# conceptofmind/vit-flax

Measured on NVIDIA B200. Metric: images/sec ViT-B/16 224 bf16 fwd at 1/2/4/8 B200; % tensor-pipe peak, higher is better.
Workload: dtype bf16

## Files before the change

vit_flax_b200/csrc/api.cu:

```cuda
#include <algorithm>
#include <cmath>
#include <cstdlib>
#include <map>
#include <memory>
#include <string>
#include <vector>

#include <cuda_fp16.h>

#include "common.h"

namespace vb {
namespace {

constexpr int DIM_HEAD = 64;

struct Leaf {
  std::string path;
  std::vector<int64_t> shape;
  float* dev = nullptr;
  bool set = false;
  int64_t numel() const {
    int64_t n = 1;
    for (auto s : shape) n *= s;
// ... 430 lines not shown
                    const AttnRecord* rec = nullptr) {
  const auto& c = m->cfg;
  const int D = c.dim, I = m->inner, T = m->T;
  const int R = batch * T;
  const ActMaps* am;
  int rc;
  if ((rc = get_act_maps(m, batch, &am))) return rc;
  const int cg_qkv = gemm_tc_tile_mode(R, 3 * I), cg_d = gemm_tc_tile_mode(R, D), cg_ff1 = gemm_tc_tile_mode(R, c.mlp_dim);
  LnFold out_a, out_b, in_a, in_b;
  out_a.x16 = out_b.x16 = m->xn_h.p;
  out_a.stats = in_a.stats = reinterpret_cast<float2*>(m->stats_a.p);
  out_b.stats = in_b.stats = reinterpret_cast<float2*>(m->stats_b.p);
  out_a.slots = out_b.slots = in_a.slots = in_b.slots = 2 * ceil_div(D, cg_d == 64 ? 64 : GEMM_BN);
  in_a.eps = in_b.eps = m->eps;
  if (m->im2col && out_a.slots % (2 * ceil_div(D, GEMM_BN)) == 0 && (reinterpret_cast<uintptr_t>(images) & 15) == 0) {
    mark(m, st, VITB200_CAT_GEMM_PATCH);
    if ((rc = patch_embed_im2col(m, st, images, batch, &out_a))) return rc;
  } else {
    mark(m, st, VITB200_CAT_PATCHIFY);
    if ((rc = launch_patchify(st, images, m->patches_h.p, batch, c.image_h, c.image_w, c.channels,
                              c.patch_h, c.patch_w, m->K0pad, m->dt, m->nchw, m->cls_off))) return rc;
    mark(m, st, VITB200_CAT_GEMM_PATCH);
    if ((rc = launch_gemm_tc(st, am->patches, m->patch.map(cg_d), &am->c_x, leaf_ptr(m, m->patch.leaf_bias), m->x.p,
                             R, D, m->K0pad, VITB200_EPI_TOKENS_LN, leaf_ptr(m, m->leaf_pos), T, m->dt, cg_d,
                             Dropout(), m->cls_off, leaf_ptr(m, m->leaf_cls), out_a))) return rc;
  }
  const bool tail = cls_tail(m, rec);
  for (int l = 0; l < c.depth; ++l) {
    Layer& L = m->layers[l];
    const bool cls_rows = tail && l + 1 == c.depth;
    const int M = cls_rows ? batch : R;
    const CUtensorMap& a_o = cls_rows ? am->o_cls : am->o;
    const CUtensorMap& c_x = cls_rows ? am->c_x_cls : am->c_x;
    mark(m, st, VITB200_CAT_GEMM_QKV);
    in_a.c = L.qkv.ln_c;
    if ((rc = launch_gemm_tc(st, am->xn, L.qkv.map_ln(cg_qkv), &am->c_qkv, L.qkv.ln_d, m->qkv_h.p, R, 3 * I, D,
                             VITB200_EPI_LN_STORE_16, nullptr, 0, m->dt, cg_qkv, Dropout(), m->cls_off, nullptr, in_a))) return rc;
    mark(m, st, VITB200_CAT_ATTENTION);
    if ((rc = attention_layer(m, st, batch, l, rec, cls_rows ? 1 : 0))) return rc;
    mark(m, st, VITB200_CAT_GEMM_OUT);
    if ((rc = launch_gemm_tc(st, a_o, L.out.map(cg_d), &c_x, leaf_ptr(m, L.out.leaf_bias), m->x.p, M, D, I,
                             VITB200_EPI_RESID_LN, nullptr, 0, m->dt, cg_d, Dropout(), m->cls_off, nullptr, out_b))) return rc;
    mark(m, st, VITB200_CAT_GEMM_FF1);
    in_b.c = L.ff1.ln_c;
    if ((rc = launch_gemm_tc(st, am->xn, L.ff1.map_ln(cg_ff1), &am->c_hid, L.ff1.ln_d, m->hid_h.p, M, c.mlp_dim, D,
                             VITB200_EPI_LN_GELU_16, nullptr, 0, m->dt, cg_ff1, Dropout(), m->cls_off, nullptr, in_b))) return rc;
    mark(m, st, VITB200_CAT_GEMM_FF2);
    if (l + 1 < c.depth) {
      if ((rc = launch_gemm_tc(st, am->h, L.ff2.map(cg_d), &am->c_x, leaf_ptr(m, L.ff2.leaf_bias), m->x.p, R, D, c.mlp_dim,
                               VITB200_EPI_RESID_LN, nullptr, 0, m->dt, cg_d, Dropout(), m->cls_off, nullptr, out_a))) return rc;
    } else {
      if ((rc = launch_gemm_tc(st, am->h, L.ff2.map(cg_d), &c_x, leaf_ptr(m, L.ff2.leaf_bias), m->x.p, M, D, c.mlp_dim,
                               VITB200_EPI_BIAS_RESID_F32, nullptr, 0, m->dt, cg_d))) return rc;
    }
  }
  return forward_head(m, st, am, batch, logits);
}

int forward_tc(vitb200_model* m, cudaStream_t st, const float* images, int batch, float* logits,
               const AttnRecord* rec = nullptr) {
  if (m->fold) return forward_tc_fold(m, st, images, batch, logits, rec);
  const auto& c = m->cfg;
  const int D = c.dim, I = m->inner, T = m->T;
  const int R = batch * T;
  const ActMaps* am;
  int rc;
  if ((rc = get_act_maps(m, batch, &am))) return rc;
  const int cgp = gemm_tc_tile_mode(R, D);
  const int cg_qkv = gemm_tc_tile_mode(R, 3 * I), cg_d = gemm_tc_tile_mode(R, D), cg_ff1 = gemm_tc_tile_mode(R, c.mlp_dim);
  const int ln_dt = m->fp8 ? VITB200_DT_E4M3 : m->dt;
  if (m->im2col && (reinterpret_cast<uintptr_t>(images) & 15) == 0) {
    mark(m, st, VITB200_CAT_GEMM_PATCH);
    if ((rc = patch_embed_im2col(m, st, images, batch, nullptr))) return rc;
  } else {
    mark(m, st, VITB200_CAT_PATCHIFY);
// ... 1232 lines not shown
```

vit_flax_b200/csrc/gemm_tc.cu:

```cuda
#include <cstdlib>

#include "common.h"
#include "ptx.cuh"

namespace vb {

namespace {

constexpr int BM = GEMM_BM, BN = GEMM_BN, BK = GEMM_BK;
constexpr int UMMA_K = 16;
constexpr int A_BYTES = BM * BK * 2;
template <int kCG> struct Cfg {
  static constexpr int CL = kCG == 64 ? 1 : kCG;
  static constexpr int BN_ = kCG == 64 ? 64 : BN;
  static constexpr int MMA_CG = CL == 1 ? 1 : 2;
  static constexpr int STAGES = kCG == 64 ? 6 : (CL == 1 ? 3 : 5);
  static constexpr int B_ROWS = BN_ / MMA_CG;
  static constexpr int B_LOAD_ROWS = BN_ / CL;
  static constexpr int B_BYTES = B_ROWS * BK * 2;
  static constexpr int STAGE_BYTES = A_BYTES + B_BYTES;
  static constexpr int TILE_M = BM * MMA_CG;
  static constexpr int PAIRS = kCG == 4 ? 2 : 1;
  static constexpr int TMEM_COLS = BN_ == 64 ? 128 : 512;
};
constexpr int NUM_EPI_WARPS = 8;
constexpr int NUM_THREADS = 128 + NUM_EPI_WARPS * 32;
constexpr int SLAB_BYTES = BM * 128;
template <int kEpi> __host__ __device__ constexpr int slabs_per_group() { return kEpi == VITB200_EPI_RESID_LN ? 3 : 2; }
template <int kCG, int kEpi> __host__ __device__ constexpr int num_stages() {
  return Cfg<kCG>::STAGES - (kEpi == VITB200_EPI_RESID_LN ? 1 : 0);
}
template <int kCG, int kEpi = VITB200_EPI_STORE_16> constexpr int smem_bytes() {
  return num_stages<kCG, kEpi>() * Cfg<kCG>::STAGE_BYTES + 2 * slabs_per_group<kEpi>() * SLAB_BYTES + 1024  +
         256 ;
}

__device__ __forceinline__ float gelu_tanh_fast(float x) {
  const float k0 = 0.7978845608028654f, k1 = 0.044715f;
  float u = k0 * x * fmaf(k1 * x, x, 1.0f);
  return 0.5f * x * (1.0f + tanh_approx(u));
}

__device__ __forceinline__ unsigned long long gelu_tanh_fast2(unsigned long long x2) {
  const unsigned long long kA = pack_f32x2(0.7978845608028654f * 0.044715f, 0.7978845608028654f * 0.044715f);
  const unsigned long long kB = pack_f32x2(0.7978845608028654f, 0.7978845608028654f);
  const unsigned long long half2 = pack_f32x2(0.5f, 0.5f);
  const unsigned long long t2 = mul_f32x2(x2, x2);
  const unsigned long long u2 = mul_f32x2(fma_f32x2(t2, kA, kB), x2);
  float u0, u1;
  unpack_f32x2(u2, u0, u1);
  const unsigned long long th2 = pack_f32x2(tanh_approx(u0), tanh_approx(u1));
  const unsigned long long hx2 = mul_f32x2(x2, half2);
  return fma_f32x2(th2, hx2, hx2);
}

template <int kEpi, int kDT, int kCG, bool kDrop, bool kMN = false>
__global__ void __launch_bounds__(NUM_THREADS, 1)
gemm_tc_kernel(const __grid_constant__ CUtensorMap tmA,
               const __grid_constant__ CUtensorMap tmB,
               const __grid_constant__ CUtensorMap tmC,
               const float* __restrict__ bias, void* __restrict__ Cout,
               int M, int N, int K, const float* __restrict__ aux, int tpi, int dbg, Dropout drop, int cls_off,
               const float* __restrict__ cls, LnFold ln, const float* __restrict__ wscale) {
  constexpr bool kF8 = (kDT == DT_E4M3);
  constexpr int kODT = kF8 ? DT_F16 : kDT;
  constexpr int KB = kF8 ? 128 : BK;
  static_assert(!kF8 || (!kMN && !kDrop), "E4M3 operands: K-major, no dropout");
  constexpr bool kOut8 = (kEpi == VITB200_EPI_BIAS_GELU_E4M3);
  constexpr bool kOut16 = (kEpi == VITB200_EPI_STORE_16 || kEpi == VITB200_EPI_BIAS_GELU_16 || kEpi == VITB200_EPI_BIAS_16 ||
                           kEpi == VITB200_EPI_BIAS_PRE_GELU_16 || kEpi == VITB200_EPI_LN_STORE_16 ||
                           kEpi == VITB200_EPI_LN_GELU_16);
  constexpr bool kLnIn = (kEpi == VITB200_EPI_LN_STORE_16 || kEpi == VITB200_EPI_LN_GELU_16);
  constexpr bool kLnOut = (kEpi == VITB200_EPI_RESID_LN || kEpi == VITB200_EPI_TOKENS_LN);
  constexpr bool kLoadX = (kEpi == VITB200_EPI_RESID_LN);
  constexpr bool kTokens = (kEpi == VITB200_EPI_TOKENS_F32 || kEpi == VITB200_EPI_TOKENS_LN);
  constexpr int SPG = slabs_per_group<kEpi>();
  constexpr bool kDual = (kEpi == VITB200_EPI_BIAS_PRE_GELU_16);
  constexpr bool kDirect = (kEpi == VITB200_EPI_PATCH_F32);
  constexpr int SLAB_COLS = (kOut16 || kOut8) ? 64 : 32;
  constexpr int SLABS_PER_TILE = Cfg<kCG>::BN_ / SLAB_COLS;
  constexpr int STAGES = num_stages<kCG, kEpi>(), B_BYTES = Cfg<kCG>::B_BYTES;
  constexpr int STAGE_BYTES = Cfg<kCG>::STAGE_BYTES, TILE_M = Cfg<kCG>::TILE_M;
  constexpr int MMA_CG = Cfg<kCG>::MMA_CG, PAIRS = Cfg<kCG>::PAIRS, CL = Cfg<kCG>::CL;
  constexpr int BN = Cfg<kCG>::BN_, TMEM_COLS = Cfg<kCG>::TMEM_COLS;
  const uint32_t crank = CL == 1 ? 0u : cluster_ctarank();
  const uint32_t rank = crank & 1u, pair = crank >> 1;
  const uint32_t lead = crank & ~1u;
  const int tile0 = int(blockIdx.x) / CL;
  const int tile_step = int(gridDim.x) / CL;

  extern __shared__ uint8_t smem_raw[];
  const uint32_t smem_base = (smem_u32(smem_raw) + 1023u) & ~1023u;
  const uint32_t sA = smem_base;
  const uint32_t sB = smem_base + STAGES * A_BYTES;
  const uint32_t sSlab = smem_base + STAGES * STAGE_BYTES;
  const uint32_t bars = sSlab + 2 * SPG * SLAB_BYTES;
  auto full_bar = [&](int s) { return bars + 8u * s; };
  auto empty_bar = [&](int s) { return bars + 8u * (STAGES + s); };
  auto tfull_bar = [&](int s) { return bars + 8u * (2 * STAGES + s); };
  auto tempty_bar = [&](int s) { return bars + 8u * (2 * STAGES + 2 + s); };
  const uint32_t tmem_slot = bars + 8u * (2 * STAGES + 4);
  auto xfull_bar = [&](int g, int b) { return bars + 8u * (2 * STAGES + 5 + g * 3 + b); };
  uint32_t* tmem_slot_ptr =
      reinterpret_cast<uint32_t*>(smem_raw + (tmem_slot - smem_u32(smem_raw)));

  const int warp = threadIdx.x >> 5;
  const int lane = threadIdx.x & 31;
  const int m_tiles = ((M + TILE_M - 1) / TILE_M + PAIRS - 1) / PAIRS;
  const int n_tiles = (N + BN - 1) / BN;
  const int num_kb = (K + KB - 1) / KB;
  const int splits = (kEpi == VITB200_EPI_BIAS_RESID_F32 && tpi > 1) ? tpi : 1;
  const int kb_per = (num_kb + splits - 1) / splits;
  const int mn_tiles = m_tiles * n_tiles;
  const int num_tiles = mn_tiles * splits;

  if (warp == 0 && lane == 0) {
    prefetch_tmap(&tmA);
    prefetch_tmap(&tmB);
    if constexpr (!kDirect) prefetch_tmap(&tmC);
  }
  if (warp == 1 && lane == 0) {
    for (int s = 0; s < STAGES; ++s) {
      mbar_init(full_bar(s), 1);
      mbar_init(empty_bar(s), PAIRS);
    }
    for (int s = 0; s < 2; ++s) {
      mbar_init(tfull_bar(s), 1);
      mbar_init(tempty_bar(s), NUM_EPI_WARPS * MMA_CG);
    }
    if constexpr (kLoadX)
      for (int i = 0; i < 6; ++i) mbar_init(xfull_bar(i / 3, i % 3), 1);
    fence_barrier_init();
  }
  if (warp == 2) tmem_alloc<MMA_CG>(tmem_slot, TMEM_COLS);
  tc_fence_before();
  if constexpr (CL != 1) cluster_sync_all(); else __syncthreads();
  tc_fence_after();
  const uint32_t tmem_base = *tmem_slot_ptr;
  pdl_launch_dependents();
  pdl_wait();

  if (warp == 0) {
    if (elect_one()) {
      int stage = 0;
      uint32_t phase = 0;
      for (int tile = tile0; tile < num_tiles; tile += tile_step) {
        const int sp = tile / mn_tiles, t2 = tile - sp * mn_tiles;
        const int m_blk = t2 / n_tiles, n_blk = t2 % n_tiles;
        const int kb0 = sp * kb_per, kb1 = min(num_kb, kb0 + kb_per);
        const int a_row = (m_blk * PAIRS + int(pair)) * TILE_M + int(rank) * BM;
        const int b_row = n_blk * BN + int(rank) * Cfg<kCG>::B_ROWS + int(pair) * Cfg<kCG>::B_LOAD_ROWS;
        for (int kb = kb0; kb < kb1; ++kb) {
          mbar_wait(empty_bar(stage), phase ^ 1u);
          if (dbg & 1) {
            if (rank == 0) mbar_arrive(full_bar(stage));
          } else if constexpr (CL == 1) {
            mbar_arrive_expect_tx(full_bar(stage), STAGE_BYTES);
            if constexpr (kMN) {
#pragma unroll
              for (int j = 0; j < BM / 64; ++j)
                tma_load_2d(sA + stage * A_BYTES + j * 8192, &tmA, full_bar(stage), a_row + j * 64, kb * BK);
#pragma unroll
              for (int j = 0; j < Cfg<kCG>::B_ROWS / 64; ++j)
// ... 52 lines not shown
          for (int k = 0; k < BK / UMMA_K; ++k) {
            if constexpr (kF8)
              umma_f8_ss<MMA_CG>(d_tmem, umma_desc_k_sw128(a0 + k * UMMA_K * 2), umma_desc_k_sw128(b0 + k * UMMA_K * 2),
                                 idesc, (kb != kb0 || k != 0) ? 1u : 0u);
            else if constexpr (kMN)
              umma_bf16_ss<MMA_CG>(d_tmem, umma_desc_mn_sw128_wide(a0 + k * UMMA_K * 128, 8192),
                                   umma_desc_mn_sw128_wide(b0 + k * UMMA_K * 128, 8192), idesc,
                                   (kb != kb0 || k != 0) ? 1u : 0u);
            else
            umma_bf16_ss<MMA_CG>(d_tmem, umma_desc_k_sw128(a0 + k * UMMA_K * 2),
                              umma_desc_k_sw128(b0 + k * UMMA_K * 2), idesc,
                              (kb != kb0 || k != 0) ? 1u : 0u);
          }
          if constexpr (CL != 1) umma_commit_cg2_mc(empty_bar(stage), all_mask);
          else umma_commit(empty_bar(stage));
          if (++stage == STAGES) { stage = 0; phase ^= 1u; }
        }
        if constexpr (CL != 1) umma_commit_cg2_mc(tfull_bar(acc), pair_mask);
        else umma_commit(tfull_bar(acc));
        acc ^= 1;
        if (acc == 0) acc_phase ^= 1u;
      }
    }
    __syncwarp();
  } else if (warp >= 4) {
    const int ew = warp - 4;
    const int q = ew & 3;
    const int grp = ew >> 2;
    const bool leader = (q == 0 && lane == 0);
    const int lrow = q * 32 + lane;
    int acc = 0;
    uint32_t acc_phase = 0;
    int buf = 0;
    int ld_tile = tile0, ld_s = grp, ld_issued = 0, x_used = 0;
    auto issue_x_load = [&]() {
      while (ld_tile < num_tiles) {
        if (ld_s < SLABS_PER_TILE && (ld_tile % n_tiles) * BN + ld_s * SLAB_COLS < N) break;
        ld_tile += tile_step;
        ld_s = grp;
      }
      if (ld_tile >= num_tiles) return;
      const int lm = ld_tile / n_tiles, lnb = ld_tile % n_tiles;
      const int b = ld_issued % 3;
      mbar_arrive_expect_tx(xfull_bar(grp, b), SLAB_BYTES);
      tma_load_2d(sSlab + uint32_t(grp * SPG + b) * SLAB_BYTES, &tmC, xfull_bar(grp, b), lnb * BN + ld_s * SLAB_COLS,
                  (lm * PAIRS + int(pair)) * TILE_M + int(rank) * BM);
      ++ld_issued;
      ld_s += 2;
    };
    if constexpr (kLoadX) {
      if (leader) { issue_x_load(); issue_x_load(); }
    }
    for (int tile = tile0; tile < num_tiles; tile += tile_step) {
      const int sp = tile / mn_tiles, t2 = tile - sp * mn_tiles;
      const int m_blk = t2 / n_tiles, n_blk = t2 % n_tiles;
      const int m_row0 = (m_blk * PAIRS + int(pair)) * TILE_M + int(rank) * BM;
      float ln_rstd = 0.f, ln_rm = 0.f;
      if constexpr (kLnIn) {
        if (m_row0 + lrow < M) {
          const float2* sp2 = ln.stats + int64_t(m_row0 + lrow) * ln.slots;
          float s1 = 0.f, s2 = 0.f;
          const float4* sp4 = reinterpret_cast<const float4*>(sp2);
          const int npair = (ln.slots & 1) ? 0 : ln.slots >> 1;
          if (ln.slots & 1) {
            for (int i = 0; i < ln.slots; ++i) { const float2 v = __ldg(sp2 + i); s1 += v.x; s2 += v.y; }
          }
          for (int i = 0; i < npair; i += 4) {
            float4 a[4];
#pragma unroll
            for (int u = 0; u < 4; ++u) a[u] = i + u < npair ? __ldg(sp4 + i + u) : make_float4(0.f, 0.f, 0.f, 0.f);
#pragma unroll
            for (int u = 0; u < 4; ++u)
              if (i + u < npair) { s1 += a[u].x; s2 += a[u].y; s1 += a[u].z; s2 += a[u].w; }
          }
          const float inv_d = 1.0f / float(K);
          const float mean = s1 * inv_d;
          ln_rstd = rsqrtf(fmaxf(s2 * inv_d - mean * mean, 0.f) + ln.eps);
          ln_rm = ln_rstd * mean;
        }
      }
      float st1 = 0.f, st2 = 0.f;
      mbar_wait(tfull_bar(acc), acc_phase);
      tc_fence_after();
      const uint32_t t_row = tmem_base + (uint32_t(q * 32) << 16) + uint32_t(acc * BN);

      if constexpr (kDirect) {
        const int row = m_row0 + lrow;
        const bool row_ok = row < M;
        const int b = row / tpi, t = row - b * tpi;
        float* crow_base = reinterpret_cast<float*>(Cout) + (int64_t(b) * (tpi + cls_off) + cls_off + t) * N;
        const float* pos_row = aux + int64_t(cls_off + t) * N;
#pragma unroll 1
        for (int chunk = 0; chunk < BN / 64; ++chunk) {
          const int n0 = n_blk * BN + grp * (BN / 2) + chunk * 32;
          if (n0 >= N) break;
          uint32_t r[32];
          tmem_ld_32x32b_x32(t_row + uint32_t(grp * (BN / 2) + chunk * 32), r);
          tmem_ld_wait();
          if (row_ok) {
#pragma unroll
            for (int j = 0; j < 8; ++j) {
              if (n0 + j * 4 < N) {
                const float4 b4 = __ldg(reinterpret_cast<const float4*>(bias + n0 + j * 4));
                const float4 p4 = __ldg(reinterpret_cast<const float4*>(pos_row + n0 + j * 4));
                float4 o;
                o.x = __uint_as_float(r[j * 4 + 0]) + b4.x + p4.x;
                o.y = __uint_as_float(r[j * 4 + 1]) + b4.y + p4.y;
                o.z = __uint_as_float(r[j * 4 + 2]) + b4.z + p4.z;
                o.w = __uint_as_float(r[j * 4 + 3]) + b4.w + p4.w;
                if constexpr (kDrop)
                  dropout4(drop, (int64_t(b) * (tpi + cls_off) + cls_off + t) * N + n0 + j * 4, o.x, o.y, o.z, o.w);
                *reinterpret_cast<float4*>(crow_base + n0 + j * 4) = o;
                if (cls != nullptr && t == 0) {
                  const float4 c4 = __ldg(reinterpret_cast<const float4*>(cls + n0 + j * 4));
                  const float4 q4 = __ldg(reinterpret_cast<const float4*>(aux + n0 + j * 4));
                  float4 z = make_float4(c4.x + q4.x, c4.y + q4.y, c4.z + q4.z, c4.w + q4.w);
                  const int64_t e0 = int64_t(b) * (tpi + 1) * N + n0 + j * 4;
                  if constexpr (kDrop) dropout4(drop, e0, z.x, z.y, z.z, z.w);
                  *reinterpret_cast<float4*>(reinterpret_cast<float*>(Cout) + e0) = z;
                }
              }
            }
          }
        }
      } else {
#pragma unroll 1
        for (int s = grp; s < SLABS_PER_TILE; s += 2) {
          const int n0 = n_blk * BN + s * SLAB_COLS;
          if (n0 >= N || (dbg & 4)) break;
          const uint32_t slab = sSlab + uint32_t(grp * SPG + (kLoadX ? x_used % 3 : buf)) * SLAB_BYTES;
          if constexpr (kLoadX) {
            mbar_wait(xfull_bar(grp, x_used % 3), uint32_t(x_used / 3) & 1u);
          } else {
            if (leader) { if constexpr (kDual) tma_store_wait_read<0>(); else tma_store_wait_read<1>(); }
            named_bar_sync(1 + grp, 128);
          }
          const uint32_t srow = slab + uint32_t(lrow) * 128u;
          const int sw = lrow & 7;
          const uint32_t srow2 = sSlab + uint32_t(grp * 2 + (buf ^ 1)) * SLAB_BYTES + uint32_t(lrow) * 128u;
          if constexpr (kOut16) {
#pragma unroll
            for (int half = 0; half < 2; ++half) {
              uint32_t r[32];
              tmem_ld_32x32b_x32(t_row + uint32_t(s * SLAB_COLS + half * 32), r);
              tmem_ld_wait();
#pragma unroll
              for (int j = 0; j < 4; ++j) {
                float v[8];
#pragma unroll
                for (int e = 0; e < 8; ++e) v[e] = __uint_as_float(r[j * 8 + e]);
                if constexpr (kF8) {
                  const int nb = n0 + half * 32 + j * 8;
                  if (nb < N) {
                    const float4 w0 = __ldg(reinterpret_cast<const float4*>(wscale + nb));
                    const float4 w1 = __ldg(reinterpret_cast<const float4*>(wscale + nb + 4));
                    v[0] *= w0.x; v[1] *= w0.y; v[2] *= w0.z; v[3] *= w0.w;
                    v[4] *= w1.x; v[5] *= w1.y; v[6] *= w1.z; v[7] *= w1.w;
                  }
                }
                if constexpr (kEpi == VITB200_EPI_BIAS_16 || kDual) {
                  const int nb = n0 + half * 32 + j * 8;
                  if (nb < N) {
                    const float4 b0 = __ldg(reinterpret_cast<const float4*>(bias + nb));
                    const float4 b1 = __ldg(reinterpret_cast<const float4*>(bias + nb + 4));
// ... 69 lines not shown
              tmem_ld_32x32b_x32(t_row + uint32_t(s * SLAB_COLS + half * 32), r);
              tmem_ld_wait();
#pragma unroll
              for (int j = 0; j < 2; ++j) {
                uint32_t q[4];
#pragma unroll
                for (int h = 0; h < 2; ++h) {
                  const int nb = n0 + half * 32 + j * 16 + h * 8;
                  float4 w0 = make_float4(0.f, 0.f, 0.f, 0.f), w1 = w0, b0 = w0, b1 = w0;
                  if (nb < N) {
                    w0 = __ldg(reinterpret_cast<const float4*>(wscale + nb));
                    w1 = __ldg(reinterpret_cast<const float4*>(wscale + nb + 4));
                    b0 = __ldg(reinterpret_cast<const float4*>(bias + nb));
                    b1 = __ldg(reinterpret_cast<const float4*>(bias + nb + 4));
                  }
                  const float ws[8] = {w0.x, w0.y, w0.z, w0.w, w1.x, w1.y, w1.z, w1.w};
                  const float bb[8] = {b0.x, b0.y, b0.z, b0.w, b1.x, b1.y, b1.z, b1.w};
                  float v[8];
#pragma unroll
                  for (int e = 0; e < 8; e += 2) {
                    const int c = j * 16 + h * 8 + e;
                    const unsigned long long y2 = fma_f32x2(pack_f32x2(__uint_as_float(r[c]), __uint_as_float(r[c + 1])),
                                                            pack_f32x2(ws[e], ws[e + 1]), pack_f32x2(bb[e], bb[e + 1]));
                    unpack_f32x2(gelu_tanh_fast2(y2), v[e], v[e + 1]);
                  }
                  q[h * 2] = pack4_e4m3(v[0], v[1], v[2], v[3]);
                  q[h * 2 + 1] = pack4_e4m3(v[4], v[5], v[6], v[7]);
                }
                const uint32_t lin = uint32_t(lrow) * 64u + uint32_t(half * 2 + j) * 16u;
                st_shared_v4(slab + (lin ^ (((lin >> 7) & 3u) << 4)), q[0], q[1], q[2], q[3]);
              }
            }
          } else {
            uint32_t r[32];
            tmem_ld_32x32b_x32(t_row + uint32_t(s * SLAB_COLS), r);
            const int tok = kTokens ? (m_row0 + lrow) % tpi : 0;
            const bool cls_row = kTokens && cls != nullptr && tok == 0;
            const float* pos_row = aux + int64_t(tok) * N;
            uint16_t* x16_row = kLnOut ? static_cast<uint16_t*>(ln.x16) + int64_t(m_row0 + lrow) * N : nullptr;
            const bool row_ok = m_row0 + lrow < M;
            uint32_t hx[8];
            tmem_ld_wait();
#pragma unroll
            for (int j = 0; j < 8; ++j) {
              const int nb = n0 + j * 4;
              float4 b4 = make_float4(0.f, 0.f, 0.f, 0.f);
              if (nb < N && sp == 0 && bias != nullptr) b4 = __ldg(reinterpret_cast<const float4*>((cls_row ? cls : bias) + nb));
              float o0 = __uint_as_float(r[j * 4 + 0]), o1 = __uint_as_float(r[j * 4 + 1]);
              float o2 = __uint_as_float(r[j * 4 + 2]), o3 = __uint_as_float(r[j * 4 + 3]);
              if constexpr (kF8) {
                if (nb < N) {
                  const float4 w4 = __ldg(reinterpret_cast<const float4*>(wscale + nb));
                  o0 *= w4.x; o1 *= w4.y; o2 *= w4.z; o3 *= w4.w;
                }
              }
              if constexpr (kTokens) {
                if (cls_row) o0 = o1 = o2 = o3 = 0.f;
                if (nb < N) {
                  const float4 p4 = __ldg(reinterpret_cast<const float4*>(pos_row + nb));
                  b4.x += p4.x; b4.y += p4.y; b4.z += p4.z; b4.w += p4.w;
                }
              }
              o0 += b4.x; o1 += b4.y; o2 += b4.z; o3 += b4.w;
              if constexpr (kDrop && kTokens)
                dropout4(drop, int64_t(m_row0 + lrow) * N + nb, o0, o1, o2, o3);
              if constexpr (kDrop && kEpi == VITB200_EPI_BIAS_RESID_F32)
                dropout4(drop, int64_t(m_row0 + lrow) * N + nb, o0, o1, o2, o3);
              if constexpr (kLoadX) {
                const float4 xo = ld_shared_v4f(srow + (uint32_t(j ^ sw) << 4));
                o0 += xo.x; o1 += xo.y; o2 += xo.z; o3 += xo.w;
              }
              st_shared_v4(srow + (uint32_t(j ^ sw) << 4), __float_as_uint(o0), __float_as_uint(o1),
                           __float_as_uint(o2), __float_as_uint(o3));
              if constexpr (kLnOut) {
                st1 += (o0 + o1) + (o2 + o3);
                st2 = fmaf(o0, o0, fmaf(o1, o1, fmaf(o2, o2, fmaf(o3, o3, st2))));
                hx[(j & 3) * 2] = pack2<kDT>(o0, o1);
                hx[(j & 3) * 2 + 1] = pack2<kDT>(o2, o3);
                if ((j & 3) == 3 && row_ok) {
                  if (nb + 4 <= N && (N & 15) == 0)
                    asm volatile("st.global.v8.b32 [%0], {%1, %2, %3, %4, %5, %6, %7, %8};" ::"l"(x16_row + nb - 12), "r"(hx[0]), "r"(hx[1]),
                                 "r"(hx[2]), "r"(hx[3]), "r"(hx[4]), "r"(hx[5]), "r"(hx[6]), "r"(hx[7]) : "memory");
                  else {
                    if (nb - 4 <= N) *reinterpret_cast<uint4*>(x16_row + nb - 12) = make_uint4(hx[0], hx[1], hx[2], hx[3]);
                    if (nb + 4 <= N) *reinterpret_cast<uint4*>(x16_row + nb - 4) = make_uint4(hx[4], hx[5], hx[6], hx[7]);
                  }
                }
              }
            }
          }
          fence_proxy_async_smem();
          named_bar_sync(1 + grp, 128);
          if (leader && !(dbg & 2)) {
            if constexpr (kEpi == VITB200_EPI_BIAS_RESID_F32)
              tma_reduce_add_2d(&tmC, slab, n0, m_row0);
            else
              tma_store_2d(&tmC, slab, n0, m_row0);
            if constexpr (kDual) tma_store_2d(&tmC, sSlab + uint32_t(grp * 2 + (buf ^ 1)) * SLAB_BYTES, n0, m_row0 + tpi);
            tma_store_commit();
          }
          if constexpr (kLoadX) {
            if (leader) { tma_store_wait_read<1>(); issue_x_load(); }
            ++x_used;
          }
          buf ^= 1;
        }
        if constexpr (kLnOut) {
          if (m_row0 + lrow < M && sp == 0)
            ln.stats[int64_t(m_row0 + lrow) * ln.slots + n_blk * 2 + grp] = make_float2(st1, st2);
        }
      }
      tc_fence_before();
      __syncwarp();
      if (lane == 0) {
        if constexpr (CL != 1) mbar_arrive_cluster(tempty_bar(acc), lead);
        else mbar_arrive(tempty_bar(acc));
      }
      acc ^= 1;
      if (acc == 0) acc_phase ^= 1u;
    }
    if (!kDirect && leader) tma_store_wait<0>();
  }

  tc_fence_before();
  if constexpr (CL != 1) cluster_sync_all(); else __syncthreads();
  if (warp == 2) {
    tc_fence_after();
    tmem_dealloc<MMA_CG>(tmem_base, TMEM_COLS);
  }
}

int gemm_dbg() {
  static int v = -1;
  if (v < 0) { const char* e = getenv("VITB200_GEMM_DBG"); v = e ? atoi(e) : 0; }
// ... 54 lines not shown
template <int kEpi, int kDT>
int launch_one(cudaStream_t stream, const CUtensorMap& tmA, const CUtensorMap& tmB,
               const CUtensorMap& tmC, const float* bias, void* C, int M, int N, int K,
               const float* aux, int tpi, int cta_group, const Dropout& drop, int cls_off, const float* cls) {
  constexpr bool kCanDrop = kEpi == VITB200_EPI_BIAS_GELU_16 || kEpi == VITB200_EPI_BIAS_RESID_F32 || kEpi == VITB200_EPI_BIAS_PRE_GELU_16 ||
                            kEpi == VITB200_EPI_PATCH_F32 || kEpi == VITB200_EPI_TOKENS_F32;
  if constexpr (kCanDrop) {
    if (drop.threshold != 0) {
      if (cta_group == 4)
        return fail(VITB200_ERR_UNSUPPORTED, "gemm_tc: dropout is not built for the opt-in cluster-of-4 mode");
      if (cta_group == 64) return launch_cg<kEpi, kDT, 64, true>(stream, tmA, tmB, tmC, bias, C, M, N, K, aux, tpi, drop, cls_off, cls);
      if (cta_group == 1) return launch_cg<kEpi, kDT, 1, true>(stream, tmA, tmB, tmC, bias, C, M, N, K, aux, tpi, drop, cls_off, cls);
      return launch_cg<kEpi, kDT, 2, true>(stream, tmA, tmB, tmC, bias, C, M, N, K, aux, tpi, drop, cls_off, cls);
    }
  }
  if (cta_group == 64) return launch_cg<kEpi, kDT, 64, false>(stream, tmA, tmB, tmC, bias, C, M, N, K, aux, tpi, drop, cls_off, cls);
  if (cta_group == 4) return launch_cg<kEpi, kDT, 4, false>(stream, tmA, tmB, tmC, bias, C, M, N, K, aux, tpi, drop, cls_off, cls);
  if (cta_group == 2) return launch_cg<kEpi, kDT, 2, false>(stream, tmA, tmB, tmC, bias, C, M, N, K, aux, tpi, drop, cls_off, cls);
  return launch_cg<kEpi, kDT, 1, false>(stream, tmA, tmB, tmC, bias, C, M, N, K, aux, tpi, drop, cls_off, cls);
}

template <int kDT>
int dispatch_epi(cudaStream_t stream, const CUtensorMap& tmA, const CUtensorMap& tmB,
                 const CUtensorMap& tmC, const float* bias, void* C, int M, int N, int K,
                 int epilogue, const float* aux, int tpi, int cta_group, const Dropout& drop, int cls_off,
                 const float* cls, const LnFold& ln) {
  if (epilogue >= VITB200_EPI_RESID_LN && epilogue <= VITB200_EPI_LN_GELU_16) {
    if (drop.threshold != 0) return fail(VITB200_ERR_UNSUPPORTED, "gemm_tc: the LayerNorm-fold epilogues have no dropout variant");
    if (ln.stats == nullptr || ln.slots <= 0) return fail(VITB200_ERR_INVALID, "gemm_tc: LayerNorm-fold epilogue without a statistics buffer");
    const bool producer = epilogue == VITB200_EPI_RESID_LN || epilogue == VITB200_EPI_TOKENS_LN;
    if (producer && (ln.x16 == nullptr || ln.slots != 2 * ceil_div(N, cta_group == 64 ? 64 : GEMM_BN)))
      return fail(VITB200_ERR_INVALID, "gemm_tc: RESID_LN / TOKENS_LN need x16 and 2 * n_tiles statistics slots");
    if (!producer && ln.c == nullptr) return fail(VITB200_ERR_INVALID, "gemm_tc: LN_STORE / LN_GELU need the column sums c");
    switch (epilogue) {
      case VITB200_EPI_RESID_LN:
        return launch_ln<VITB200_EPI_RESID_LN, kDT>(stream, tmA, tmB, tmC, bias, C, M, N, K, aux, 0, cta_group, cls_off, cls, ln);
      case VITB200_EPI_TOKENS_LN:
        if (aux == nullptr || tpi <= 0) return fail(VITB200_ERR_INVALID, "gemm_tc: TOKENS_LN needs pos_embedding and tokens per image");
        return launch_ln<VITB200_EPI_TOKENS_LN, kDT>(stream, tmA, tmB, tmC, bias, C, M, N, K, aux, tpi, cta_group, cls_off, cls, ln);
      case VITB200_EPI_LN_STORE_16:
        return launch_ln<VITB200_EPI_LN_STORE_16, kDT>(stream, tmA, tmB, tmC, bias, C, M, N, K, aux, 0, cta_group, cls_off, cls, ln);
      default:
        return launch_ln<VITB200_EPI_LN_GELU_16, kDT>(stream, tmA, tmB, tmC, bias, C, M, N, K, aux, 0, cta_group, cls_off, cls, ln);
    }
  }
  switch (epilogue) {
    case VITB200_EPI_STORE_16:
      return launch_one<VITB200_EPI_STORE_16, kDT>(stream, tmA, tmB, tmC, bias, C, M, N, K, aux, tpi, cta_group, drop, cls_off, cls);
    case VITB200_EPI_BIAS_GELU_16:
      return launch_one<VITB200_EPI_BIAS_GELU_16, kDT>(stream, tmA, tmB, tmC, bias, C, M, N, K, aux, tpi, cta_group, drop, cls_off, cls);
    case VITB200_EPI_BIAS_RESID_F32:
      return launch_one<VITB200_EPI_BIAS_RESID_F32, kDT>(stream, tmA, tmB, tmC, bias, C, M, N, K, aux, tpi, cta_group, drop, cls_off, cls);
    case VITB200_EPI_BIAS_F32:
      return launch_one<VITB200_EPI_BIAS_F32, kDT>(stream, tmA, tmB, tmC, bias, C, M, N, K, aux, tpi, cta_group, drop, cls_off, cls);
    case VITB200_EPI_PATCH_F32:
      if (aux == nullptr || tpi <= 0)
        return fail(VITB200_ERR_INVALID, "gemm_tc: PATCH epilogue needs pos_embedding and tokens");
      return launch_one<VITB200_EPI_PATCH_F32, kDT>(stream, tmA, tmB, tmC, bias, C, M, N, K, aux, tpi, cta_group, drop, cls_off, cls);
    case VITB200_EPI_BIAS_16:
      return launch_one<VITB200_EPI_BIAS_16, kDT>(stream, tmA, tmB, tmC, bias, C, M, N, K, aux, tpi, cta_group, drop, cls_off, cls);
    case VITB200_EPI_BIAS_PRE_GELU_16:
      if (tpi < M) return fail(VITB200_ERR_INVALID, "gemm_tc: PRE_GELU epilogue needs the row offset of its second output (>= M)");
      return launch_one<VITB200_EPI_BIAS_PRE_GELU_16, kDT>(stream, tmA, tmB, tmC, bias, C, M, N, K, aux, tpi, cta_group, drop, cls_off, cls);
    case VITB200_EPI_TOKENS_F32:
      if (aux == nullptr || tpi <= 0)
        return fail(VITB200_ERR_INVALID, "gemm_tc: TOKENS epilogue needs pos_embedding and tokens per image");
      return launch_one<VITB200_EPI_TOKENS_F32, kDT>(stream, tmA, tmB, tmC, bias, C, M, N, K, aux, tpi, cta_group, drop, cls_off, cls);
    default:
      return fail(VITB200_ERR_INVALID, "gemm_tc: unknown epilogue");
// ... 105 lines not shown
```

vit_flax_b200/csrc/ptx.cuh:

```cuda
#pragma once
#include <cuda_runtime.h>
#include <cuda_bf16.h>
#include <cuda_fp16.h>
#include <stdint.h>
#include <stdio.h>

namespace vb {

__device__ __forceinline__ uint32_t smem_u32(const void* p) {
  return static_cast<uint32_t>(__cvta_generic_to_shared(p));
}
__device__ __forceinline__ uint32_t lane_id() { return threadIdx.x & 31u; }
__device__ __forceinline__ bool elect_one() {
  uint32_t pred;
  asm volatile("{\n\t.reg .pred p;\n\telect.sync _|p, 0xffffffff;\n\tselp.u32 %0, 1, 0, p;\n\t}" : "=r"(pred));
  return pred != 0;
}

__device__ __forceinline__ void pdl_wait() { asm volatile("griddepcontrol.wait;" ::: "memory"); }
__device__ __forceinline__ void pdl_launch_dependents() {
  asm volatile("griddepcontrol.launch_dependents;" ::: "memory");
}

__device__ __forceinline__ void mbar_init(uint32_t bar, uint32_t count) {
// ... 122 lines not shown
      " [%0], [%1, {%3, %4, %5}], [%2];"
      ::"r"(dst), "l"(reinterpret_cast<uint64_t>(tmap)), "r"(bar), "r"(c0), "r"(c1), "r"(c2)
      : "memory");
}
__device__ __forceinline__ void tma_load_im2col_5d(uint32_t dst, const void* tmap, uint32_t bar, int32_t c, int32_t w,
                                                   int32_t h, int32_t d, int32_t n, uint16_t w_off, uint16_t h_off,
                                                   uint16_t d_off) {
  asm volatile(
      "cp.async.bulk.tensor.5d.shared::cluster.global.im2col.mbarrier::complete_tx::bytes"
      " [%0], [%1, {%3, %4, %5, %6, %7}], [%2], {%8, %9, %10};"
      ::"r"(dst), "l"(reinterpret_cast<uint64_t>(tmap)), "r"(bar), "r"(c), "r"(w), "r"(h), "r"(d), "r"(n), "h"(w_off),
        "h"(h_off), "h"(d_off)
      : "memory");
}
__device__ __forceinline__ void tma_store_commit() { asm volatile("cp.async.bulk.commit_group;" ::: "memory"); }
template <int N>
__device__ __forceinline__ void tma_store_wait_read() {
  asm volatile("cp.async.bulk.wait_group.read %0;" ::"n"(N) : "memory");
}
template <int N>
__device__ __forceinline__ void tma_store_wait() {
  asm volatile("cp.async.bulk.wait_group %0;" ::"n"(N) : "memory");
}
__device__ __forceinline__ void named_bar_sync(uint32_t id, uint32_t nthreads) {
  asm volatile("bar.sync %0, %1;" ::"r"(id), "r"(nthreads) : "memory");
}
__device__ __forceinline__ float4 ld_shared_v4f(uint32_t addr) {
  float4 v;
  asm volatile("ld.shared.v4.f32 {%0, %1, %2, %3}, [%4];" : "=f"(v.x), "=f"(v.y), "=f"(v.z), "=f"(v.w) : "r"(addr) : "memory");
  return v;
}
__device__ __forceinline__ void st_shared_v4(uint32_t addr, uint32_t a, uint32_t b, uint32_t c, uint32_t d) {
  asm volatile("st.shared.v4.b32 [%0], {%1, %2, %3, %4};" ::"r"(addr), "r"(a), "r"(b), "r"(c), "r"(d) : "memory");
}

template <int kCtaGroup>
__device__ __forceinline__ void tmem_alloc(uint32_t smem_dst, uint32_t ncols) {
  if constexpr (kCtaGroup == 1) {
    asm volatile("tcgen05.alloc.cta_group::1.sync.aligned.shared::cta.b32 [%0], %1;"
                 ::"r"(smem_dst), "r"(ncols) : "memory");
    asm volatile("tcgen05.relinquish_alloc_permit.cta_group::1.sync.aligned;" ::: "memory");
  } else {
    asm volatile("tcgen05.alloc.cta_group::2.sync.aligned.shared::cta.b32 [%0], %1;"
                 ::"r"(smem_dst), "r"(ncols) : "memory");
    asm volatile("tcgen05.relinquish_alloc_permit.cta_group::2.sync.aligned;" ::: "memory");
  }
}
template <int kCtaGroup>
__device__ __forceinline__ void tmem_dealloc(uint32_t taddr, uint32_t ncols) {
  if constexpr (kCtaGroup == 1)
    asm volatile("tcgen05.dealloc.cta_group::1.sync.aligned.b32 %0, %1;" ::"r"(taddr), "r"(ncols)
                 : "memory");
  else
    asm volatile("tcgen05.dealloc.cta_group::2.sync.aligned.b32 %0, %1;" ::"r"(taddr), "r"(ncols)
                 : "memory");
}
__device__ __forceinline__ void tc_fence_before() {
  asm volatile("tcgen05.fence::before_thread_sync;" ::: "memory");
}
__device__ __forceinline__ void tc_fence_after() {
  asm volatile("tcgen05.fence::after_thread_sync;" ::: "memory");
}

template <int kCtaGroup>
__device__ __forceinline__ void umma_bf16_ss(uint32_t d_tmem, uint64_t adesc, uint64_t bdesc,
                                             uint32_t idesc, uint32_t accumulate) {
// ... 226 lines not shown
  uint32_t site = 0;
  uint32_t threshold = 0;
  float inv_keep = 1.f;
};
__device__ __forceinline__ uint4 philox4x32_10(unsigned long long quad, uint32_t site, uint32_t k0, uint32_t k1) {
  uint32_t c0 = uint32_t(quad), c1 = uint32_t(quad >> 32), c2 = site, c3 = 0u;
#pragma unroll
  for (int r = 0; r < 10; ++r) {
    const uint32_t hi0 = __umulhi(0xD2511F53u, c0), lo0 = 0xD2511F53u * c0;
    const uint32_t hi1 = __umulhi(0xCD9E8D57u, c2), lo1 = 0xCD9E8D57u * c2;
    c0 = hi1 ^ c1 ^ k0;
    c1 = lo1;
    c2 = hi0 ^ c3 ^ k1;
    c3 = lo0;
    k0 += 0x9E3779B9u;
    k1 += 0xBB67AE85u;
  }
  return make_uint4(c0, c1, c2, c3);
}
__device__ __forceinline__ void dropout4(const Dropout& d, long long elem, float& a, float& b, float& c, float& e) {
  const uint4 r = philox4x32_10(static_cast<unsigned long long>(elem) >> 2, d.site, d.key_lo, d.key_hi);
  a = r.x < d.threshold ? 0.f : a * d.inv_keep;
  b = r.y < d.threshold ? 0.f : b * d.inv_keep;
  c = r.z < d.threshold ? 0.f : c * d.inv_keep;
  e = r.w < d.threshold ? 0.f : e * d.inv_keep;
}

struct LnFold {
  void* x16 = nullptr;
  float2* stats = nullptr;
  const float* c = nullptr;
  int slots = 0;
  float eps = 1e-6f;
};

__device__ __forceinline__ float tanh_approx(float x) {
  float y;
  asm("tanh.approx.f32 %0, %1;" : "=f"(y) : "f"(x));
  return y;
}
__device__ __forceinline__ float ex2_approx(float x) {
  float y;
  asm("ex2.approx.ftz.f32 %0, %1;" : "=f"(y) : "f"(x));
  return y;
}

}
```

Before: 28770.

## Prefetch residual x into registers for large-K RESID_LN GEMM epilogue

New measurement: 28990 (median of 6 runs). No clear change (+0.8%).

```diff
diff --git a/profiles/run_resid_ln.py b/profiles/run_resid_ln.py
--- /dev/null
+++ b/profiles/run_resid_ln.py
@@ -0,0 +1,78 @@
+import argparse
+import ctypes as C
+import hashlib
+import json
+import sys
+from pathlib import Path
+
+import torch
+
+ap = argparse.ArgumentParser()
+ap.add_argument("--tree", default=str(Path(__file__).resolve().parents[1]))
+ap.add_argument("--reps", type=int, default=50)
+ap.add_argument("--dtype", default="bf16", choices=["bf16", "fp16"])
+ap.add_argument("--check", action="store_true")
+args = ap.parse_args()
+
+sys.path.insert(0, str(Path(args.tree).resolve()))
+from vit_flax_b200 import _lib
+
+lib = _lib.load()
+dt = _lib.DT_BF16 if args.dtype == "bf16" else _lib.DT_F16
+tdt = torch.bfloat16 if args.dtype == "bf16" else torch.float16
+st = C.c_void_p(torch.cuda.current_stream().cuda_stream)
+
+TIMED = [(50432, 768, 768, "to_out"), (50432, 768, 3072, "ff2")]
+CHECKED = TIMED + [(12608, 1280, 1024, "vit_h_width"), (1000, 328, 256, "ragged"), (256, 768, 768, "mode_64"),
+                   (200, 256, 512, "mode_1")]
+
+
+def setup(M, N, K, seed=0):
+    g = torch.Generator(device="cuda").manual_seed(seed)
+    A = torch.randn((M, K), device="cuda", generator=g).to(tdt)
+    Wt = (torch.randn((N, K), device="cuda", generator=g) / K ** 0.5).to(tdt)
+    bias = torch.randn(N, device="cuda", generator=g)
+    x = torch.randn((M, N), device="cuda", generator=g)
+    x16 = torch.empty((M, N), device="cuda", dtype=tdt)
+    slots = lib.vitb200_gemm_tc_ln_slots(M, N)
+    stats = torch.zeros((M, slots, 2), device="cuda")
+    return A, Wt, bias, x, x16, stats, slots
+
+
+def launch(M, N, K, A, Wt, bias, x, x16, stats, slots):
+    _lib.check(lib.vitb200_gemm_tc_ln(st, A.data_ptr(), Wt.data_ptr(), bias.data_ptr(), x.data_ptr(), M, N, K,
+                                      _lib.EPI_RESID_LN, None, 0, None, dt, x16.data_ptr(), stats.data_ptr(), slots,
+                                      None, 0.0))
+
+
+def digest(t):
+    return hashlib.sha256(t.contiguous().view(torch.uint8).cpu().numpy().tobytes()).hexdigest()[:16]
+
+
+if args.check:
+    for M, N, K, name in CHECKED:
+        bufs = setup(M, N, K)
+        launch(M, N, K, *bufs)
+        torch.cuda.synchronize()
+        _, _, _, x, x16, stats, _ = bufs
+        print(json.dumps({"shape": name, "M": M, "N": N, "K": K, "x": digest(x), "x16": digest(x16),
+                          "stats": digest(stats)}))
+    sys.exit(0)
+
+for M, N, K, name in TIMED:
+    bufs = setup(M, N, K)
+    for _ in range(5):
+        launch(M, N, K, *bufs)
+    torch.cuda.synchronize()
+    e0, e1 = torch.cuda.Event(enable_timing=True), torch.cuda.Event(enable_timing=True)
+    e0.record()
+    for _ in range(args.reps):
+        launch(M, N, K, *bufs)
+    e1.record()
+    torch.cuda.synchronize()
+    us = e0.elapsed_time(e1) * 1e3 / args.reps
+    slots = bufs[-1]
+    nbytes = 2 * M * K + 2 * N * K + 4 * M * N * 2 + 2 * M * N + 8 * M * slots
+    print(json.dumps({"shape": name, "M": M, "N": N, "K": K, "dtype": args.dtype, "reps": args.reps,
+                      "us": round(us, 2), "tflops": round(2 * M * N * K / us / 1e6, 1),
+                      "gbps": round(nbytes / us / 1e3, 1), "tree": args.tree}))
diff --git a/vit_flax_b200/csrc/api.cu b/vit_flax_b200/csrc/api.cu
--- a/vit_flax_b200/csrc/api.cu
+++ b/vit_flax_b200/csrc/api.cu
@@ -486,6 +486,8 @@
     const int M = cls_rows ? batch : R;
     const CUtensorMap& a_o = cls_rows ? am->o_cls : am->o;
     const CUtensorMap& c_x = cls_rows ? am->c_x_cls : am->c_x;
+    LnFold out_o = out_b;
+    if (cls_rows) out_o.x_pitch = T * D;
     mark(m, st, VITB200_CAT_GEMM_QKV);
     in_a.c = L.qkv.ln_c;
     if ((rc = launch_gemm_tc(st, am->xn, L.qkv.map_ln(cg_qkv), &am->c_qkv, L.qkv.ln_d, m->qkv_h.p, R, 3 * I, D,
@@ -494,7 +496,7 @@
     if ((rc = attention_layer(m, st, batch, l, rec, cls_rows ? 1 : 0))) return rc;
     mark(m, st, VITB200_CAT_GEMM_OUT);
     if ((rc = launch_gemm_tc(st, a_o, L.out.map(cg_d), &c_x, leaf_ptr(m, L.out.leaf_bias), m->x.p, M, D, I,
-                             VITB200_EPI_RESID_LN, nullptr, 0, m->dt, cg_d, Dropout(), m->cls_off, nullptr, out_b))) return rc;
+                             VITB200_EPI_RESID_LN, nullptr, 0, m->dt, cg_d, Dropout(), m->cls_off, nullptr, out_o))) return rc;
     mark(m, st, VITB200_CAT_GEMM_FF1);
     in_b.c = L.ff1.ln_c;
     if ((rc = launch_gemm_tc(st, am->xn, L.ff1.map_ln(cg_ff1), &am->c_hid, L.ff1.ln_d, m->hid_h.p, M, c.mlp_dim, D,
diff --git a/vit_flax_b200/csrc/gemm_tc.cu b/vit_flax_b200/csrc/gemm_tc.cu
--- a/vit_flax_b200/csrc/gemm_tc.cu
+++ b/vit_flax_b200/csrc/gemm_tc.cu
@@ -26,14 +26,17 @@
 constexpr int NUM_EPI_WARPS = 8;
 constexpr int NUM_THREADS = 128 + NUM_EPI_WARPS * 32;
 constexpr int SLAB_BYTES = BM * 128;
-template <int kEpi> __host__ __device__ constexpr int slabs_per_group() { return kEpi == VITB200_EPI_RESID_LN ? 3 : 2; }
-template <int kCG, int kEpi> __host__ __device__ constexpr int num_stages() {
-  return Cfg<kCG>::STAGES - (kEpi == VITB200_EPI_RESID_LN ? 1 : 0);
-}
-template <int kCG, int kEpi = VITB200_EPI_STORE_16> constexpr int smem_bytes() {
+constexpr int EPI_RESID_LN_RING = 100 + VITB200_EPI_RESID_LN;
+constexpr int RESID_LN_REG_MIN_K = 2048;
+template <int kEpi> __host__ __device__ constexpr int slabs_per_group() { return kEpi == EPI_RESID_LN_RING ? 3 : 2; }
+template <int kCG, int kEpi> __host__ __device__ constexpr int num_stages() { return Cfg<kCG>::STAGES - (kEpi == EPI_RESID_LN_RING ? 1 : 0); }
+template <int kCG, int kEpi> constexpr int smem_bytes() {
   return num_stages<kCG, kEpi>() * Cfg<kCG>::STAGE_BYTES + 2 * slabs_per_group<kEpi>() * SLAB_BYTES + 1024  +
          256 ;
 }
+static_assert(smem_bytes<1, 0>() <= 227 * 1024 && smem_bytes<2, 0>() <= 227 * 1024 && smem_bytes<4, 0>() <= 227 * 1024 &&
+              smem_bytes<64, 0>() <= 227 * 1024 && smem_bytes<2, EPI_RESID_LN_RING>() <= 227 * 1024,
+              "gemm_tc: shared memory over the 227 KB a block may have");
 
 __device__ __forceinline__ float gelu_tanh_fast(float x) {
   const float k0 = 0.7978845608028654f, k1 = 0.044715f;
@@ -71,7 +74,8 @@
                            kEpi == VITB200_EPI_BIAS_PRE_GELU_16 || kEpi == VITB200_EPI_LN_STORE_16 ||
                            kEpi == VITB200_EPI_LN_GELU_16);
   constexpr bool kLnIn = (kEpi == VITB200_EPI_LN_STORE_16 || kEpi == VITB200_EPI_LN_GELU_16);
-  constexpr bool kLnOut = (kEpi == VITB200_EPI_RESID_LN || kEpi == VITB200_EPI_TOKENS_LN);
+  constexpr bool kRing = (kEpi == EPI_RESID_LN_RING);
+  constexpr bool kLnOut = (kEpi == VITB200_EPI_RESID_LN || kRing || kEpi == VITB200_EPI_TOKENS_LN);
   constexpr bool kLoadX = (kEpi == VITB200_EPI_RESID_LN);
   constexpr bool kTokens = (kEpi == VITB200_EPI_TOKENS_F32 || kEpi == VITB200_EPI_TOKENS_LN);
   constexpr int SPG = slabs_per_group<kEpi>();
@@ -128,7 +132,7 @@
       mbar_init(tfull_bar(s), 1);
       mbar_init(tempty_bar(s), NUM_EPI_WARPS * MMA_CG);
     }
-    if constexpr (kLoadX)
+    if constexpr (kRing)
       for (int i = 0; i < 6; ++i) mbar_init(xfull_bar(i / 3, i % 3), 1);
     fence_barrier_init();
   }
@@ -247,23 +251,53 @@
     int acc = 0;
     uint32_t acc_phase = 0;
     int buf = 0;
-    int ld_tile = tile0, ld_s = grp, ld_issued = 0, x_used = 0;
-    auto issue_x_load = [&]() {
+    float xc[32], xn[32];
+    int ld_tile = tile0, ld_s = grp;
+    const int64_t x_pitch = ln.x_pitch > 0 ? ln.x_pitch : N;
+    auto load_next_x = [&]() {
       while (ld_tile < num_tiles) {
         if (ld_s < SLABS_PER_TILE && (ld_tile % n_tiles) * BN + ld_s * SLAB_COLS < N) break;
         ld_tile += tile_step;
         ld_s = grp;
       }
       if (ld_tile >= num_tiles) return;
-      const int lm = ld_tile / n_tiles, lnb = ld_tile % n_tiles;
-      const int b = ld_issued % 3;
-      mbar_arrive_expect_tx(xfull_bar(grp, b), SLAB_BYTES);
-      tma_load_2d(sSlab + uint32_t(grp * SPG + b) * SLAB_BYTES, &tmC, xfull_bar(grp, b), lnb * BN + ld_s * SLAB_COLS,
-                  (lm * PAIRS + int(pair)) * TILE_M + int(rank) * BM);
-      ++ld_issued;
+      const int lm = ld_tile / n_tiles, c0 = (ld_tile % n_tiles) * BN + ld_s * SLAB_COLS;
+      const int row = (lm * PAIRS + int(pair)) * TILE_M + int(rank) * BM + lrow;
+      const float* src = static_cast<const float*>(Cout) + int64_t(row) * x_pitch + c0;
+#pragma unroll
+      for (int p = 0; p < 4; ++p) {
+        if (row < M && c0 + p * 8 < N) {
+          ld_global_v8f(src + p * 8, xn + p * 8);
+        } else {
+#pragma unroll
+          for (int e = 0; e < 8; ++e) xn[p * 8 + e] = 0.f;
+        }
+      }
       ld_s += 2;
     };
-    if constexpr (kLoadX) {
+    auto advance_x = [&]() {
+#pragma unroll
+      for (int e = 0; e < 32; ++e) xc[e] = xn[e];
+      load_next_x();
+    };
+    if constexpr (kLoadX) load_next_x();
+    int rg_tile = tile0, rg_s = grp, rg_issued = 0, x_used = 0;
+    auto issue_x_load = [&]() {
+      while (rg_tile < num_tiles) {
+        if (rg_s < SLABS_PER_TILE && (rg_tile % n_tiles) * BN + rg_s * SLAB_COLS < N) break;
+        rg_tile += tile_step;
+        rg_s = grp;
+      }
+      if (rg_tile >= num_tiles) return;
+      const int lm = rg_tile / n_tiles, lnb = rg_tile % n_tiles;
+      const int b = rg_issued % 3;
+      mbar_arrive_expect_tx(xfull_bar(grp, b), SLAB_BYTES);
+      tma_load_2d(sSlab + uint32_t(grp * SPG + b) * SLAB_BYTES, &tmC, xfull_bar(grp, b), lnb * BN + rg_s * SLAB_COLS,
+                  (lm * PAIRS + int(pair)) * TILE_M + int(rank) * BM);
+      ++rg_issued;
+      rg_s += 2;
+    };
+    if constexpr (kRing) {
       if (leader) { issue_x_load(); issue_x_load(); }
     }
     for (int tile = tile0; tile < num_tiles; tile += tile_step) {
@@ -295,6 +329,9 @@
         }
       }
       float st1 = 0.f, st2 = 0.f;
+      if constexpr (kLoadX) {
+        if (n_blk * BN + grp * SLAB_COLS < N) advance_x();
+      }
       mbar_wait(tfull_bar(acc), acc_phase);
       tc_fence_after();
       const uint32_t t_row = tmem_base + (uint32_t(q * 32) << 16) + uint32_t(acc * BN);
@@ -343,8 +380,11 @@
         for (int s = grp; s < SLABS_PER_TILE; s += 2) {
           const int n0 = n_blk * BN + s * SLAB_COLS;
           if (n0 >= N || (dbg & 4)) break;
-          const uint32_t slab = sSlab + uint32_t(grp * SPG + (kLoadX ? x_used % 3 : buf)) * SLAB_BYTES;
           if constexpr (kLoadX) {
+            if (s != grp) advance_x();
+          }
+          const uint32_t slab = sSlab + uint32_t(grp * SPG + (kRing ? x_used % 3 : buf)) * SLAB_BYTES;
+          if constexpr (kRing) {
             mbar_wait(xfull_bar(grp, x_used % 3), uint32_t(x_used / 3) & 1u);
           } else {
             if (leader) { if constexpr (kDual) tma_store_wait_read<0>(); else tma_store_wait_read<1>(); }
@@ -480,8 +520,10 @@
               }
             }
           } else {
-            uint32_t r[32];
-            tmem_ld_32x32b_x32(t_row + uint32_t(s * SLAB_COLS), r);
+            constexpr int RC = kLoadX ? 16 : 32;
+            uint32_t r[RC];
+            if constexpr (kLoadX) tmem_ld_32x32b_x16(t_row + uint32_t(s * SLAB_COLS), r);
+            else tmem_ld_32x32b_x32(t_row + uint32_t(s * SLAB_COLS), r);
             const int tok = kTokens ? (m_row0 + lrow) % tpi : 0;
             const bool cls_row = kTokens && cls != nullptr && tok == 0;
             const float* pos_row = aux + int64_t(tok) * N;
@@ -492,10 +534,16 @@
 #pragma unroll
             for (int j = 0; j < 8; ++j) {
               const int nb = n0 + j * 4;
+              if (kLoadX && j == 4) {
+                __syncwarp();
+                tmem_ld_32x32b_x16(t_row + uint32_t(s * SLAB_COLS + 16), r);
+                tmem_ld_wait();
+              }
+              const int jr = j % (RC / 4);
               float4 b4 = make_float4(0.f, 0.f, 0.f, 0.f);
               if (nb < N && sp == 0 && bias != nullptr) b4 = __ldg(reinterpret_cast<const float4*>((cls_row ? cls : bias) + nb));
-              float o0 = __uint_as_float(r[j * 4 + 0]), o1 = __uint_as_float(r[j * 4 + 1]);
-              float o2 = __uint_as_float(r[j * 4 + 2]), o3 = __uint_as_float(r[j * 4 + 3]);
+              float o0 = __uint_as_float(r[jr * 4 + 0]), o1 = __uint_as_float(r[jr * 4 + 1]);
+              float o2 = __uint_as_float(r[jr * 4 + 2]), o3 = __uint_as_float(r[jr * 4 + 3]);
               if constexpr (kF8) {
                 if (nb < N) {
                   const float4 w4 = __ldg(reinterpret_cast<const float4*>(wscale + nb));
@@ -515,6 +563,9 @@
               if constexpr (kDrop && kEpi == VITB200_EPI_BIAS_RESID_F32)
                 dropout4(drop, int64_t(m_row0 + lrow) * N + nb, o0, o1, o2, o3);
               if constexpr (kLoadX) {
+                o0 += xc[j * 4 + 0]; o1 += xc[j * 4 + 1]; o2 += xc[j * 4 + 2]; o3 += xc[j * 4 + 3];
+              }
+              if constexpr (kRing) {
                 const float4 xo = ld_shared_v4f(srow + (uint32_t(j ^ sw) << 4));
                 o0 += xo.x; o1 += xo.y; o2 += xo.z; o3 += xo.w;
               }
@@ -547,7 +598,7 @@
             if constexpr (kDual) tma_store_2d(&tmC, sSlab + uint32_t(grp * 2 + (buf ^ 1)) * SLAB_BYTES, n0, m_row0 + tpi);
             tma_store_commit();
           }
-          if constexpr (kLoadX) {
+          if constexpr (kRing) {
             if (leader) { tma_store_wait_read<1>(); issue_x_load(); }
             ++x_used;
           }
@@ -668,9 +719,13 @@
     if (producer && (ln.x16 == nullptr || ln.slots != 2 * ceil_div(N, cta_group == 64 ? 64 : GEMM_BN)))
       return fail(VITB200_ERR_INVALID, "gemm_tc: RESID_LN / TOKENS_LN need x16 and 2 * n_tiles statistics slots");
     if (!producer && ln.c == nullptr) return fail(VITB200_ERR_INVALID, "gemm_tc: LN_STORE / LN_GELU need the column sums c");
+    if (epilogue == VITB200_EPI_RESID_LN && ((reinterpret_cast<uintptr_t>(C) & 31) != 0 || ln.x_pitch % 8 != 0))
+      return fail(VITB200_ERR_INVALID, "gemm_tc: RESID_LN reads x_old in 32-byte pieces: C must be 32-byte aligned, its row pitch a multiple of 8");
     switch (epilogue) {
       case VITB200_EPI_RESID_LN:
-        return launch_ln<VITB200_EPI_RESID_LN, kDT>(stream, tmA, tmB, tmC, bias, C, M, N, K, aux, 0, cta_group, cls_off, cls, ln);
+        if (K >= RESID_LN_REG_MIN_K)
+          return launch_ln<VITB200_EPI_RESID_LN, kDT>(stream, tmA, tmB, tmC, bias, C, M, N, K, aux, 0, cta_group, cls_off, cls, ln);
+        return launch_ln<EPI_RESID_LN_RING, kDT>(stream, tmA, tmB, tmC, bias, C, M, N, K, aux, 0, cta_group, cls_off, cls, ln);
       case VITB200_EPI_TOKENS_LN:
         if (aux == nullptr || tpi <= 0) return fail(VITB200_ERR_INVALID, "gemm_tc: TOKENS_LN needs pos_embedding and tokens per image");
         return launch_ln<VITB200_EPI_TOKENS_LN, kDT>(stream, tmA, tmB, tmC, bias, C, M, N, K, aux, tpi, cta_group, cls_off, cls, ln);
diff --git a/vit_flax_b200/csrc/ptx.cuh b/vit_flax_b200/csrc/ptx.cuh
--- a/vit_flax_b200/csrc/ptx.cuh
+++ b/vit_flax_b200/csrc/ptx.cuh
@@ -178,6 +178,11 @@
 }
 __device__ __forceinline__ void st_shared_v4(uint32_t addr, uint32_t a, uint32_t b, uint32_t c, uint32_t d) {
   asm volatile("st.shared.v4.b32 [%0], {%1, %2, %3, %4};" ::"r"(addr), "r"(a), "r"(b), "r"(c), "r"(d) : "memory");
+}
+__device__ __forceinline__ void ld_global_v8f(const float* p, float* v) {
+  asm volatile("ld.global.L1::no_allocate.v8.f32 {%0, %1, %2, %3, %4, %5, %6, %7}, [%8];"
+               : "=f"(v[0]), "=f"(v[1]), "=f"(v[2]), "=f"(v[3]), "=f"(v[4]), "=f"(v[5]), "=f"(v[6]), "=f"(v[7])
+               : "l"(p) : "memory");
 }
 
 template <int kCtaGroup>
@@ -470,6 +475,7 @@
   const float* c = nullptr;
   int slots = 0;
   float eps = 1e-6f;
+  int x_pitch = 0;
 };
 
 __device__ __forceinline__ float tanh_approx(float x) {
```
